# tuffy/libdvd-audio

Measured on AMD Instinct MI355X. Metric: decoded PCM Msamples/s (bit-exact) on 6ch/96k/24b MLP, higher is better.
Workload: dtype int32 (int64 accumulate)

## Files before the change

### libdvd-audio_amd/csrc/mlp_decode.h

```cpp
#pragma once
#include <hip/hip_runtime.h>
#if defined(__HIP_DEVICE_COMPILE__) && !defined(__gfx950__)
#error "mlp_decode.h is written for gfx950 (MI355X): hand-placed s_waitcnt encodings and gfx950 inline asm"
#endif
#include <stdint.h>
#include <type_traits>
#include "mlp_bounds.h"
#include "mlp_index.h"
#include "mlp_tables.h"

namespace mlp {

constexpr int DEC_THREADS = 128;
constexpr int DEC_WAVES = DEC_THREADS / 64;
constexpr int MAXCH = 8;
constexpr int MAXMAT = 6;
constexpr int RING_PLANES = 8;
constexpr int RING_DWORDS = RING_PLANES * 4;
constexpr int CHUNK_DWORDS = 16;
constexpr int OUT_ROWS = 4;
constexpr uint32_t YIELD_LONELY = 48;
#ifndef DVDA_HDR_GATE_TURNS
#define DVDA_HDR_GATE_TURNS 32
#endif
// ... 210 lines not shown

template <int RD>
__device__ __forceinline__ void ring_store4(uint32_t *dst, const uint4 &a, bool first_plane)
{
    const uint32_t a0 = be32(a.x);
    if (first_plane)
        dst[-RD * 64] = a0;
    dst[0] = a0;
    dst[-1 * 64] = be32(a.y);
    dst[-2 * 64] = be32(a.z);
    dst[-3 * 64] = be32(a.w);
}

__device__ __forceinline__ void ring_fill_sync(const uint4 *src, uint32_t *dst, bool first_plane)
{
    const uint4 a = src[0], b = src[1], c = src[2], d = src[3];
    ring_store16(dst, a, b, c, d, first_plane);
}

__device__ __attribute__((noinline)) int64_t iir_mac(const int32_t *ws, uint32_t stride)
{
    int64_t acc = 0;
    for (uint32_t j = 0; j < 8; j++)
        acc += (int64_t)ws[(size_t)j * stride] * (int64_t)ws[(size_t)(8 + j) * stride];
    return acc;
}

__device__ __attribute__((noinline)) void iir_push(int32_t *ws, uint32_t stride, int32_t v)
{
    for (int j = 7; j > 0; j--)
        ws[(size_t)(8 + j) * stride] = ws[(size_t)(8 + j - 1) * stride];
    ws[(size_t)8 * stride] = v;
}

template <int RD, int G>
struct BitReaderT {
    const uint4 *gsrc;
    uint32_t *ring;
    uint32_t max_chunk;
    uint32_t pos;
    uint32_t fillpos;
    uint32_t lo_valid;

    __device__ __forceinline__ uint32_t *slot(uint32_t d) const
    {
        return ring + ((RD - (d & (RD - 1))) << 6);
    }
    __device__ __forceinline__ uint64_t window() const
    {
        const uint32_t *p = ring + ((~(pos >> 5) & (RD - 1)) << 6);
        return ((uint64_t)p[64] << 32) | p[0];
    }
    __device__ __forceinline__ uint32_t window_lds() const
    {
        return (uint32_t)(uintptr_t)ring + ((~(pos >> 5) & (RD - 1)) << 8);
    }
    __device__ __forceinline__ int32_t ahead() const
    {
        return (int32_t)((fillpos << 5) - (pos & ~31u)) >> 5;
    }
    __device__ __forceinline__ void filled()
    {
        fillpos += G;
        if (fillpos - lo_valid > (uint32_t)RD)
            lo_valid = fillpos - RD;
    }
    __device__ __forceinline__ uint32_t fill_src() const
    {
        const uint32_t last = max_chunk + (uint32_t)(CHUNK_DWORDS - G);
        return fillpos < last ? fillpos : last;
    }
    __device__ __forceinline__ bool room() const { return ahead() <= (int32_t)(RD - G); }
    __device__ __forceinline__ void fill_sync()
    {
        if constexpr (G == CHUNK_DWORDS) {
            ring_fill_sync(gsrc + (fill_src() >> 2), slot(fillpos), (fillpos & (RD - 1)) == 0);
            filled();
        } else {
            uint4 q[4];
            const int32_t n = fill_issue(q);
            fill_commit(q, n);
        }
    }
    __device__ __forceinline__ int32_t fill_issue(uint4 (&q)[4]) const
    {
        static_assert(G == CHUNK_DWORDS || (G == 4 && RD == 16), "the small ring is 16 dwords filled by 16-byte granules");
        const int32_t n = room() ? (RD - ahead()) >> 2 : 0;
#pragma unroll
        for (int g = 0; g < 4; g++)
            if (g < n) {
                const uint32_t f = fillpos + 4u * g, last = max_chunk + (uint32_t)(CHUNK_DWORDS - G);
                q[g] = gsrc[(f < last ? f : last) >> 2];
            }
        return n;
    }
    __device__ __forceinline__ void fill_commit(const uint4 (&q)[4], int32_t n)
    {
#pragma unroll
        for (int g = 0; g < 4; g++)
            if (g < n) {
                ring_store4<RD>(slot(fillpos), q[g], (fillpos & (RD - 1)) == 0);
                filled();
            }
    }
    __device__ __forceinline__ void ensure(uint32_t n)
    {
#if defined(DVDA_EXP_STAMP)
        const unsigned long long t0_ = clock64();
        bool any_ = false;
#endif
        while (__builtin_expect(__any(ahead() < (int32_t)n), 0)) {
            if (room())
                fill_sync();
#if defined(DVDA_EXP_STAMP)
            any_ = true;
#endif
        }
#if defined(DVDA_EXP_STAMP)
        if (any_) {
            fill_cyc += clock64() - t0_;
            fill_n++;
        }
#endif
    }
#if defined(DVDA_EXP_STAMP)
    unsigned long long fill_cyc = 0, fill_n = 0;
#endif
    __device__ __forceinline__ void seek_byte(uint64_t byte_pos)
    {
        const uint32_t t = (uint32_t)(byte_pos >> 2);
        if (!((int32_t)(t - lo_valid) >= 0 && (int32_t)(fillpos - t) > 0)) {
            fillpos = t & ~(uint32_t)(G - 1);
            lo_valid = fillpos;
        }
        pos = (uint32_t)byte_pos << 3;
    }
    __device__ __forceinline__ uint64_t tell_near(uint64_t ref_bits) const
    {
        return ref_bits + (uint64_t)(int64_t)(int32_t)(pos - (uint32_t)ref_bits);
    }
    __device__ __forceinline__ bool past(uint32_t end_bits_lo) const { return (int32_t)(pos - end_bits_lo) > 0; }
    __device__ __forceinline__ uint32_t peek32()
    {
        ensure(2);
        return (uint32_t)((window() << (pos & 31u)) >> 32);
    }
    __device__ __forceinline__ uint32_t read(uint32_t n)
    {
        const uint32_t top = peek32();
        pos += n;
        return n ? top >> (32 - n) : 0u;
    }
    __device__ __forceinline__ uint32_t read_resident(uint32_t n)
    {
        const uint32_t top = (uint32_t)((window() << (pos & 31u)) >> 32);
        pos += n;
        return (top >> 1) >> (31u - n);
    }
    __device__ __forceinline__ int32_t read_signed_resident(uint32_t n)
    {
        const uint32_t top = (uint32_t)((window() << (pos & 31u)) >> 32);
        pos += n;
        return n ? (int32_t)top >> ((32u - n) & 31u) : 0;
    }
    __device__ __forceinline__ int32_t read_signed(uint32_t n)
    {
        if (n == 0)
            return 0;
        const int32_t v = (int32_t)peek32() >> (32 - n);
        pos += n;
        return v;
    }
};

using BitReader = BitReaderT<RING_DWORDS, CHUNK_DWORDS>;
constexpr int DUO_RING = 16, DUO_GRAN = 4;

__device__ __forceinline__ uint32_t huff_decode_m(uint32_t cb, uint32_t t, uint64_t m_esc, uint32_t bmask)
{
    const uint32_t a = (((t & 0xFFu) >> (5u + cb)) + 7u) | ((4u - cb) << 8);
    const uint32_t z = (uint32_t)__clz((int)((t << 25) | 0x01000000u));
    const uint32_t base = __builtin_amdgcn_ubfe(0x08090B08u, 8u * cb, 8u);
    uint32_t up = base + z, dn = 6u - z;
    asm volatile("" : "+v"(up), "+v"(dn));
    uint32_t val = (t & 0x80u) ? up : dn;
    val = z > 6u ? 0xFFu : val;
    uint32_t e = val | (((z > 6u ? 6u : z) + 3u) << 8);
    asm("v_cndmask_b32_e64 %0, %0, %1, %2" : "+v"(e) : "v"(a), "s"(m_esc));
    return e & bmask;
}

__device__ __forceinline__ uint32_t huff_decode(uint32_t cb, uint32_t t)
{
    uint64_t m_esc = __builtin_amdgcn_ballot_w64((t & 0x100u) != 0);
    asm volatile("" : "+s"(m_esc));
    return huff_decode_m(cb, t, m_esc, cb ? 0xFFFFFFFFu : 0u);
}

struct SubPark {
    uint32_t flags, block_size, min_ch, max_ch, max_mat_ch, noise_shift, seed, matrix_len, bypass_mask, outch_pack,
             oshift_pack, qss_pack, nslots, iir_any, ss_end_bit, rows_left, blocks_in_frame, chk, gl, seg_lane;
    bool have_restart, seg_iir;
    uint32_t *brec, *brec_end, *brec_base;
};

template <int NS, bool PAIRED, bool GENERAL, bool ILV = false, bool PARSE = false, bool DUO = false, bool WAVO = false>
__global__ __launch_bounds__(DEC_THREADS, 2) void k_decode(DecodeArgs a)
{
    static_assert(!(GENERAL && PARSE), "one mode at a time");
    static_assert(!DUO || (!PAIRED && !GENERAL && NS == 6), "the two-substream lane is a one-lane fast-pass / parse instance");
    static_assert(GENERAL == PAIRED, "lane pairs are the sequential pass's layout, and its only one");
    constexpr uint32_t L = PAIRED ? 2u : 1u;
    if (!GENERAL && a.only_S && a.cls[a.only_S - 1u] == 0)
        return;
    if (!GENERAL && !PARSE && coop_takes(a))
        return;
    constexpr int THREADS = DEC_THREADS;
    constexpr int WAVES = THREADS / 64;
    constexpr int TP = 6;
    constexpr int RD = DUO ? DUO_RING : RING_DWORDS;
    constexpr int RG = DUO ? DUO_GRAN : CHUNK_DWORDS;
    using Reader = BitReaderT<RD, RG>;
    __shared__ uint32_t s_ring[WAVES][DUO ? 2 : 1][RD + 1][64];
    __shared__ int32_t s_out[GENERAL ? 1 : WAVES][TP][OUT_ROWS][GENERAL ? 1 : 64];
    constexpr bool XCH = PAIRED;
    __shared__ int32_t s_xch[XCH ? WAVES : 1][MAXCH][XCH ? 64 : 1];
    __shared__ uint32_t s_nchained[WAVES];

    if (threadIdx.x < WAVES)
        s_nchained[threadIdx.x] = 0;
    __syncthreads();

    const int lane = threadIdx.x & 63;
    const int wv = threadIdx.x >> 6;
    const uint32_t wg_id = blockIdx.x;
    const uint32_t gl0 = wg_id * THREADS + threadIdx.x;
    uint32_t n_seg = *a.n_seg_ptr;
    if (n_seg > a.max_seg)
        n_seg = a.max_seg;
    const uint32_t item = gl0 / L;
    uint32_t segi = item;
    bool active = segi < n_seg;
    if (!GENERAL && !PARSE && active && *a.hetero)
        segi = DVDA_AT(a.lane_seg, item, a.caps.max_seg, BT_LANE_SEG);
    if (!GENERAL && !PARSE && segi >= n_seg) {
        active = false;
        segi = n_seg;
    }
    if (GENERAL || PARSE) {
        active = item < a.list_n && (a.list_n_ptr == nullptr || item < *a.list_n_ptr) && (!PARSE || item < DVDA_AT(a.plan, n_seg, a.caps.max_seg + 1u, BT_PLAN).y);
        segi = 0;
        if (active) {
            const uint32_t e = DVDA_AT(a.list, a.list_base + item, GENERAL ? a.caps.max_streams : a.caps.max_seg, BT_LIST);
            segi = GENERAL ? DVDA_AT(a.streams, e, a.caps.max_streams, BT_STREAMS).first_seg : e;
            active = segi < n_seg;
        }
        if (!active)
            segi = n_seg;
    }

    SegRec sr;
    sr.off = sr.end = 0;
    sr.stream = 0;
    sr.nframes = 0;
    sr.flags = 0;
    sr.sync = 0;
    sr.ndrop = 0;
    sr.prev = 0xFFFFFFFFu;
    uint32_t fbase = 0, stream_sync = 0, stream_first = 0;
    if (active) {
        sr = DVDA_AT(a.seg, segi, a.caps.max_seg, BT_SEG);
        stream_first = DVDA_AT(a.streams, sr.stream, a.caps.max_streams, BT_STREAMS).first_seg;
        if (stream_first == 0xFFFFFFFFu) {
            active = false;
            stream_first = segi;
        } else {
            stream_sync = a.streams[sr.stream].sync;
            fbase = a.seg_fbase[segi] - DVDA_AT(a.seg_fbase, stream_first, a.caps.max_seg + 1u, BT_FBASE);
        }
    }
    const uint32_t S = (stream_sync >> 24) & 0xF;
    const uint32_t sub = DUO ? 1u : gl0 - item * L;
    uint32_t gl = segi * 2u + sub;
    uint32_t seg_lane = gl;
    const uint32_t assignment = (stream_sync >> 16) & 0x1F;
    const uint32_t rpa = rows_per_au((stream_sync >> 8) & 0xF);
    const uint32_t nch_out = channel_count(assignment);
    const uint32_t wavepk = wave_pack(assignment);
    const uint32_t wave_inv = ILV ? wave_inv_pack(assignment) : 0u;
    uint32_t status = 0;
    if (active && (sr.flags & ST_FATAL_INDEX))
        active = false;
    if (active && (sub >= S || sr.nframes == 0))
        active = false;
    bool mine = GENERAL || !a.only_S || S == a.only_S;
    if (!mine)
        active = false;
    if (active && S > (DUO ? 2u : L)) {
        status |= ST_ENVELOPE;
        active = false;
    }
    if (DUO && S != 2u)
        active = false;
    if (active && (rpa == 0 || nch_out == 0)) {
        status |= ST_ENVELOPE;
        active = false;
    }
    const bool is_last_sub = (sub + 1 == S);
    const bool owner = is_last_sub;

// ... 62 lines not shown
        const uint64_t edge = out_stride < row_limit ? out_stride : row_limit;
        if (edge > row0)
            room = edge - row0 > 0xFFFFFFFFull ? 0xFFFFFFFFu : (uint32_t)(edge - row0);
    }
    const bool vec_ok = PARSE || ((((out_base | out_stride) & 3) == 0) &&
                                  ((reinterpret_cast<uintptr_t>(a.pcm) & 15) == 0));
    bool dir_ok = true;
    if (ILV && !GENERAL && !PARSE && segi < n_seg) {
        const uint64_t ob = a.out_off[sr.stream], os = a.out_stride[sr.stream];
        dir_ok = nch_out == 6u && (wavepk & 0xFFFFFFu) == 0x543210u && ((ob | os) & 3) == 0 &&
                 (reinterpret_cast<uintptr_t>(a.pcm) & 15) == 0;
    }
    const bool ilv_direct = ILV && !GENERAL && !PARSE && __all(dir_ok);

    Reader rd;
    rd.gsrc = reinterpret_cast<const uint4 *>(a.bytes);
    rd.ring = &s_ring[wv][DUO ? 1 : 0][0][lane];
    rd.max_chunk = (uint32_t)(((a.total_bytes + 63) >> 6) << 4);
    rd.pos = 0;
    rd.fillpos = 0;
    rd.lo_valid = 0;
    uint32_t chk = active ? DVDA_AT(a.seg_check, (size_t)segi * 2u + sub, 2ull * a.caps.max_seg, BT_CHECK) : 0xFFFFFFFFu;
    Reader rx;
    rx.gsrc = rd.gsrc;
    rx.ring = &s_ring[wv][0][0][lane];
    rx.max_chunk = rd.max_chunk;
    rx.pos = 0;
    rx.fillpos = 0;
    rx.lo_valid = 0;
    SubPark P0;
    P0.flags = 0xFF;
    P0.block_size = 8;
    P0.min_ch = P0.max_ch = P0.max_mat_ch = P0.noise_shift = P0.seed = P0.matrix_len = P0.bypass_mask = P0.outch_pack = 0;
    P0.oshift_pack = P0.qss_pack = P0.nslots = P0.iir_any = P0.ss_end_bit = P0.rows_left = P0.blocks_in_frame = 0;
    P0.have_restart = false;
    P0.seg_iir = false;
    P0.gl = segi * 2u;
    P0.seg_lane = P0.gl;
    P0.chk = (DUO && active) ? DVDA_AT(a.seg_check, (size_t)segi * 2u, 2ull * a.caps.max_seg, BT_CHECK) : 0xFFFFFFFFu;
    P0.brec = P0.brec_end = P0.brec_base = nullptr;
    if (DUO && PARSE && active) {
        const uint4 pl = DVDA_AT(a.plan, segi, a.caps.max_seg + 1u, BT_PLAN);
        P0.brec = a.brec + brec_offset(pl.x, pl.y, 0u, seg_R);
        P0.brec_base = P0.brec;
        P0.brec_end = P0.brec + brec_capacity(seg_R);
        if (!DVDA_RANGE_OK(brec_offset(pl.x, pl.y, 0u, seg_R), brec_capacity(seg_R), a.caps.brec, BT_BREC)) {
            status |= ST_CAPACITY;
            active = false;
        }
    }

    uint64_t sp[NS][4];
    auto st_get = [&](int k, int j) -> int32_t {
        return (j & 1) ? (int32_t)(uint32_t)(sp[k][j >> 1] >> 32) : (int32_t)(uint32_t)sp[k][j >> 1];
    };
    auto st_set = [&](int k, int j, int32_t v) {
        if (j & 1)
            sp[k][j >> 1] = (sp[k][j >> 1] & 0xFFFFFFFFull) | ((uint64_t)(uint32_t)v << 32);
        else
            sp[k][j >> 1] = (sp[k][j >> 1] & 0xFFFFFFFF00000000ull) | (uint32_t)v;
    };
    constexpr bool CFU = !PARSE && !GENERAL && !DUO;
    constexpr int CFW = CFU ? 8 : 4;
    int32_t cf[NS][CFW];
    uint32_t pk[NS];
    int32_t sho[NS];
    uint32_t mreg[2][4];
    uint32_t mnoise[2] = {0, 0};
    constexpr bool MU = ILV && !PAIRED && !GENERAL && !PARSE && !DUO;
    int32_t mu[2][MU ? 8 : 1];
#pragma unroll
    for (int m = 0; m < 2; m++)
#pragma unroll
        for (int j = 0; j < (MU ? 8 : 1); j++)
            mu[m][j] = 0;
#pragma unroll
    for (int k = 0; k < NS; k++) {
#pragma unroll
        for (int j = 0; j < 4; j++)
            sp[k][j] = 0;
#pragma unroll
        for (int j = 0; j < CFW; j++)
            cf[k][j] = 0;
        pk[k] = 24u << 2;
        sho[k] = -(1 << 23);
    }
#pragma unroll
    for (int m = 0; m < 2; m++)
#pragma unroll
        for (int j = 0; j < 4; j++)
            mreg[m][j] = 0;
    if (GENERAL && resume_from_init) {
#pragma unroll
        for (int k = 0; k < NS; k++)
#pragma unroll
            for (int j = 0; j < 8; j++)
                st_set(k, j, a.init_fir[((size_t)sr.stream * 2 + sub) * 48 + k * 8 + j]);
    }
    uint32_t flags = 0xFF;
    uint32_t block_size = 8;
    uint32_t min_ch = 0, max_ch = 0, max_mat_ch = 0, noise_shift = 0, seed = 0;
    uint32_t matrix_len = 0, bypass_mask = 0, outch_pack = 0;
    uint32_t oshift_pack = 0, qss_pack = 0;
    uint32_t qss_A = 0, mmc_A = 0;
    uint32_t gate_turn = 0;
    auto no_restart_yet = [&]() -> uint32_t {
        if (GENERAL)
            return ST_ENVELOPE;
        const uint32_t first = a.streams[a.seg[segi].stream].first_seg;
        return segi != first ? ST_SEQ : ST_ENVELOPE;
    };
    constexpr bool HDR_GATE = !PAIRED && !GENERAL;
    const uint32_t gl_r = gl;
    uint32_t nslots = 0;
    bool have_restart = false;
    uint32_t iir_any = 0;
    bool seg_iir = false;

    uint64_t cur = sr.off;
    uint32_t ss_end_bit = 0;
    uint32_t rows_left = 0;
    bool in_frame = false;
    uint32_t frame_rows = 0;
    uint32_t blocks_in_frame = 0;
    uint32_t frames_done = 0;
    uint64_t row = row0;
    uint32_t rows_written = 0;
    uint32_t rows_done = 0;
    int32_t pq_s[OUT_ROWS] = {0, 0, 0, 0};
    uint32_t au_idx = 0;
    uint32_t drops_seen = 0;
    uint32_t dsub = sub;
    auto swap_sub = [&]() {
        auto sw = [](uint32_t &x, uint32_t &y) { const uint32_t t = x; x = y; y = t; };
        auto swb = [](bool &x, bool &y) { const bool t = x; x = y; y = t; };
        auto swp = [](uint32_t *&x, uint32_t *&y) { uint32_t *const t = x; x = y; y = t; };
        sw(rd.pos, rx.pos);
        sw(rd.fillpos, rx.fillpos);
        sw(rd.lo_valid, rx.lo_valid);
        swp(rd.ring, rx.ring);
        sw(flags, P0.flags);
        sw(block_size, P0.block_size);
        sw(min_ch, P0.min_ch);
        sw(max_ch, P0.max_ch);
        sw(max_mat_ch, P0.max_mat_ch);
        sw(noise_shift, P0.noise_shift);
        sw(seed, P0.seed);
        sw(matrix_len, P0.matrix_len);
        sw(bypass_mask, P0.bypass_mask);
        sw(outch_pack, P0.outch_pack);
        sw(oshift_pack, P0.oshift_pack);
        sw(qss_pack, P0.qss_pack);
        sw(nslots, P0.nslots);
        sw(iir_any, P0.iir_any);
        sw(ss_end_bit, P0.ss_end_bit);
        sw(rows_left, P0.rows_left);
        sw(blocks_in_frame, P0.blocks_in_frame);
        sw(chk, P0.chk);
        sw(gl, P0.gl);
        sw(seg_lane, P0.seg_lane);
        swb(have_restart, P0.have_restart);
        swb(seg_iir, P0.seg_iir);
        swp(brec, P0.brec);
        swp(brec_end, P0.brec_end);
        swp(brec_base, P0.brec_base);
        dsub ^= 1u;
    };
// ... 342 lines not shown
                                            a.mat_ws[(size_t)(m * 5 + (c >> 1)) * a.total_lanes + gl] = word;
#pragma unroll
                                            for (int mm = 0; mm < 2; mm++)
#pragma unroll
                                                for (int jj = 0; jj < 4; jj++)
                                                    if ((uint32_t)mm == m && (uint32_t)jj == (c >> 1) && mat_mine) {
                                                        mreg[mm][jj] = word;
                                                        if constexpr (MU) {
                                                            if (jj < 3) {
                                                                mu[mm][MU ? 2 * jj : 0] = lo16(word);
                                                                mu[mm][MU ? 2 * jj + 1 : 0] = hi16(word);
                                                            }
                                                        }
                                                    }
                                        }
                                    } else {
                                        pair = (uint32_t)vc & 0xFFFFu;
                                    }
                                }
                                a.mat_ws[(size_t)(m * 5 + 4) * a.total_lanes + gl] = noise;
                                if (m == 0 && mat_mine)
                                    mnoise[0] = noise;
                                if (m == 1 && mat_mine)
                                    mnoise[1] = noise;
                                if constexpr (MU) {
#pragma unroll
                                    for (int mm = 0; mm < 2; mm++)
                                        if ((uint32_t)mm == m && mat_mine) {
                                            mu[mm][MU ? 6 : 0] = lo16(noise);
                                            mu[mm][MU ? 7 : 0] = hi16(noise);
                                        }
                                }
                            }
                        } else if (restart) {
                            matrix_len = 0;
                            bypass_mask = 0;
                        }
                        if (ok && (flags & 0x04u) && rd.read_resident(1)) {
                            if (blocks_in_frame)
                                matrix_class_change = true;
                            for (uint32_t c = 0; c <= max_mat_ch; c++) {
                                const int32_t v = rd.read_signed_resident(4);
                                if (v < 0) {
                                    ok = false;
                                    err = ST_ENVELOPE;
                                }
                                oshift_pack = (oshift_pack & ~(0xFu << (4 * c))) | (((uint32_t)v & 0xFu) << (4 * c));
                            }
                        } else if (restart) {
                            oshift_pack = 0;
                        }
                        bool qss_changed = false;
                        if (ok && (flags & 0x08u) && rd.read_resident(1)) {
                            if (blocks_in_frame)
                                matrix_class_change = true;
                            for (uint32_t c = 0; c <= max_ch; c++)
                                qss_pack = (qss_pack & ~(0xFu << (4 * c))) | (rd.read_resident(4) << (4 * c));
                            qss_changed = true;
                        } else if (restart) {
                            qss_pack = 0;
                            qss_changed = true;
                        }
                        DVDA_HSTAMP(2);
                        for (uint32_t k = 0; k < nslots && ok; k++) {
                            rd.ensure(HDR_FIR);
                            const uint32_t c = min_ch + k;
                            const uint32_t kr = DUO ? c : k;
                            uint32_t pk_old = 0;
                            int32_t sho_old = 0;
                            uint32_t cf_old[4] = {0, 0, 0, 0};
#pragma unroll
                            for (int kk = 0; kk < NS; kk++)
                                if ((uint32_t)kk == kr) {
                                    pk_old = pk[kk];
                                    sho_old = sho[kk];
                                    if (PARSE) {
#pragma unroll
                                        for (int j = 0; j < 4; j++)
                                            cf_old[j] = !CFU ? (uint32_t)cf[kk][CFU ? 0 : j]
                                                             : (((uint32_t)cf[kk][CFU ? 2 * j : 0] & 0xFFFFu) |
                                                                ((uint32_t)cf[kk][CFU ? 2 * j + 1 : 0] << 16));
                                    }
                                }
                            uint32_t codebook = pk_old & 3u;
                            const uint32_t lb_old = (pk_old >> 2) & 31u, q_old = (pk_old >> 7) & 15u;
                            uint32_t iir_order = (pk_old >> 15) & 0xFu, fir_order = (pk_old >> 19) & 0xFu;
                            uint32_t fir_shift = (pk_old >> 23) & 0xFu, iir_shift = (pk_old >> 27) & 0xFu;
                            uint32_t lsbs = lb_old + q_old;
                            int32_t hoff = sho_old + huff_center(codebook, lb_old);
                            bool touched = qss_changed;
                            bool new_fir = false, new_iir = false;
                            uint32_t ncf[4] = {0, 0, 0, 0};
                            if (rd.read_resident(1)) {
                                touched = true;
                                if ((flags & 0x10u) && rd.read_resident(1)) {
                                    fir_order = rd.read_resident(4);
                                    new_fir = true;
                                    if (fir_order > 8) {
                                        ok = false;
                                    } else if (fir_order == 0) {
                                        fir_shift = 0;
                                    } else {
                                        fir_shift = rd.read_resident(4);
                                        const uint32_t cbits = rd.read_resident(5);
                                        const uint32_t cshift = rd.read_resident(3);
                                        if (cbits < 1 || cbits > 16 || cbits + cshift > 16) {
                                            ok = false;
                                        } else {
#pragma unroll
                                            for (int j = 0; j < 8; j++) {
                                                int32_t v = 0;
                                                if ((uint32_t)j < fir_order)
                                                    v = (int32_t)((uint32_t)rd.read_signed_resident(cbits) << cshift);
                                                if (j & 1)
                                                    ncf[j >> 1] |= (uint32_t)v << 16;
                                                else
                                                    ncf[j >> 1] = (uint32_t)v & 0xFFFFu;
                                            }
                                            if (rd.read_resident(1))
                                                ok = false;
                                        }
                                    }
                                } else if (restart) {
                                    fir_order = 0;
                                    fir_shift = 0;
                                    new_fir = true;
                                }
                                rd.ensure(HDR_IIR);
                                if (ok && (flags & 0x20u) && rd.read_resident(1)) {
                                    new_iir = true;
                                    iir_order = rd.read_resident(4);
                                    if (iir_order > 8) {
                                        ok = false;
                                    } else if (iir_order == 0) {
                                        iir_shift = 0;
                                    } else {
                                        iir_shift = rd.read_resident(4);
                                        const uint32_t cbits = rd.read_resident(5);
                                        const uint32_t cshift = rd.read_resident(3);
                                        if (cbits < 1 || cbits > 16 || cbits + cshift > 16) {
                                            ok = false;
                                        } else {
                                            int32_t *ws = a.iir_ws + (size_t)(k * 16) * a.total_lanes + gl;
                                            for (uint32_t j = 0; j < 8; j++) {
                                                int32_t v = 0;
                                                if (j < iir_order)
                                                    v = (int32_t)((uint32_t)rd.read_signed_resident(cbits) << cshift);
                                                ws[(size_t)j * a.total_lanes] = v;
                                            }
                                            rd.ensure(HDR_IIR_STATE);
                                            if (rd.read_resident(1)) {
                                                const uint32_t sbits = rd.read_resident(4), sshift = rd.read_resident(4);
                                                if (sbits == 0) {
                                                    ok = false;
                                                    err = ST_ENVELOPE;
                                                }
                                                for (uint32_t j = 0; j < 8; j++) {
                                                    int32_t v = 0;
                                                    if (j < iir_order)
                                                        v = (int32_t)((uint32_t)rd.read_signed_resident(sbits) << sshift);
                                                    ws[(size_t)(8 + j) * a.total_lanes] = v;
                                                }
                                            } else {
                                                ok = false;
                                                err = ST_ENVELOPE;
                                            }
                                        }
                                    }
                                } else if (restart) {
                                    new_iir = true;
                                    iir_order = 0;
                                    iir_shift = 0;
                                }
                                if (ok && (flags & 0x40u) && rd.read_resident(1))
                                    hoff = rd.read_signed_resident(15);
                                else if (restart)
                                    hoff = 0;
                                codebook = rd.read_resident(2);
                                lsbs = rd.read_resident(5);
                                if (lsbs > 24)
                                    ok = false;
                            } else if (restart) {
                                touched = true;
                                fir_order = fir_shift = iir_order = iir_shift = 0;
                                new_fir = true;
                                new_iir = true;
                                hoff = 0;
                                codebook = 0;
                                lsbs = 24;
                            }
                            if (touched && ok) {
                                const uint32_t q = nib(qss_pack, c);
                                if (lsbs < q) {
                                    ok = false;
                                    err = ST_ENVELOPE;
                                } else {
                                    const uint32_t lb = lsbs - q;
                                    uint32_t shift;
                                    if (fir_order + iir_order > 8) {
                                        ok = false;
                                        err = ST_FILTER;
                                    }
                                    if (fir_shift > 0 && iir_shift > 0) {
                                        if (fir_shift != iir_shift) {
                                            ok = false;
                                            err = ST_FILTER;
                                        }
                                        shift = fir_shift;
                                    } else if (fir_order > 0) {
                                        shift = fir_shift;
                                    } else {
                                        shift = iir_shift;
                                    }
                                    if (fir_order && frames_done == 0 && blocks_in_frame == 0)
                                        status |= ST_CHAINED;
                                    const int32_t nsho = hoff - huff_center(codebook, lb);
                                    const uint32_t npk = codebook | (lb << 2) | (q << 7) | (shift << 11) |
                                                         (iir_order << 15) | (fir_order << 19) |
                                                         (fir_shift << 23) | (iir_shift << 27) |
                                                         (codebook ? 1u << 31 : 0u);
#pragma unroll
                                    for (int kk = 0; kk < NS; kk++)
                                        if ((uint32_t)kk == kr) {
                                            pk[kk] = npk;
                                            sho[kk] = nsho;
                                            if (new_fir) {
#pragma unroll
                                                for (int j = 0; j < 4; j++) {
                                                    if constexpr (!CFU) {
                                                        cf[kk][CFU ? 0 : j] = (int32_t)ncf[j];
                                                    } else {
                                                        cf[kk][CFU ? 2 * j : 0] = lo16(ncf[j]);
                                                        cf[kk][CFU ? 2 * j + 1 : 0] = hi16(ncf[j]);
                                                    }
                                                }
                                            }
                                        }
                                    iir_any = (iir_any & ~(1u << k)) | ((iir_order ? 1u : 0u) << k);
                                    if (PARSE) {
                                        const bool with_iir = new_iir && iir_order != 0;
                                        if (brec + 2 * BREC_STRIDE + (with_iir ? BREC_IIR_WORDS : 0) > brec_end) {
                                            seq_needed = true;
                                        } else {
                                            uint32_t *w = brec + BREC_SLOT * k;
                                            w[2] = shift | (q << 4) | (fir_order << 8) | (iir_order << 12) |
                                                   (new_iir ? 1u << 16 : 0u);
#pragma unroll
                                            for (int j = 0; j < 4; j++)
                                                w[3 + j] = new_fir ? ncf[j] : cf_old[j];
                                            w[7] = 0;
                                            chg_mask |= 1u << k;
                                            if (with_iir) {
                                                const int32_t *ws = a.iir_ws + (size_t)(k * 16) * a.total_lanes + gl;
                                                brec_end -= BREC_IIR_WORDS;
                                                uint32_t *x = brec_end;
                                                for (uint32_t j = 0; j < 4; j++)
                                                    x[j] = ((uint32_t)ws[(size_t)(2 * j) * a.total_lanes] & 0xFFFFu) |
                                                           ((uint32_t)ws[(size_t)(2 * j + 1) * a.total_lanes] << 16);
                                                for (uint32_t j = 0; j < 8; j++)
                                                    x[4 + j] = (uint32_t)ws[(size_t)(8 + j) * a.total_lanes];
                                                w[7] = (uint32_t)(x - brec_base);
                                            }
                                        }
                                    }
                                }
                            }
                        }
                    }
                }
                DVDA_HSTAMP(3);
                if (!have_restart && ok) {
                    ok = false;
                    err = no_restart_yet();
                }
                hdr_parsed = true;
                if (PARSE && iir_any)
                    seg_iir = true;
                if (PARSE && ok && chg_mask) {
#pragma unroll
                    for (int kk = 0; kk < 6; kk++) {
                        brec[BREC_SLOT * kk] = rows_done;
                        brec[BREC_SLOT * kk + 1] = (chg_mask >> kk) & 1u;
                    }
                    brec += BREC_STRIDE;
                }
                if (PARSE && ok && (seq_needed || (hdr_restart && blocks_in_frame))) {
                    status |= ST_SEQ;
                    active = false;
                }
                if (mat_mine) {
                    qss_A = qss_pack;
                    mmc_A = max_mat_ch;
                }
                const uint32_t cold_ml = matrix_len;
                if (matrix_class_change)
                    status |= ST_MIDFRAME;
                if (!ok) {
                    status |= err;
                    active = false;
                } else if (PARSE && !active) {
                } else if (!GENERAL && !PARSE && (iir_any != 0 || cold_ml > 2)) {
                    status |= ST_COLD;
                    active = false;
                } else if (!GENERAL && !PARSE && (status & ST_CHAINED)) {
                    active = false;
                    if (!(DUO && probe))
                        atomicAdd(&s_nchained[wv], 1u);
                    if (sr.prev != 0xFFFFFFFFu)
                        __hip_atomic_store(&DVDA_AT(a.yield_req, sr.prev, a.caps.max_seg, BT_YIELD), 1u, __ATOMIC_RELAXED, __HIP_MEMORY_SCOPE_AGENT);
                } else {
                    rows_left = block_size;
                    blocks_in_frame++;
                    if (!GENERAL && !PARSE && frames_done < 2 &&
                        __hip_atomic_load(&s_nchained[wv], __ATOMIC_RELAXED, __HIP_MEMORY_SCOPE_WORKGROUP) >= YIELD_LONELY) {
                        status |= ST_YIELD;
                        active = false;
                    }
                }
            }
                if constexpr (DUO) {
                    if (pass == 0u && me)
                        swap_sub();
                    if (!PARSE && pass == 0u && me && !active && first0 && !(status & ~ST_INFO)) {
                        probe = true;
                        active = true;
                    }
                    if (pass == 1u && probe)
                        active = false;
                }
            }
            if constexpr (DUO) {
                if (active && have_restart && P0.have_restart && (P0.min_ch != 0u || min_ch != P0.max_ch + 1u)) {
                    status |= PARSE ? ST_SEQ : ST_COLD;
                    active = false;
                }
            }
        }
        if (hdr_now) {
            DVDA_HSTAMP(4);
#if defined(DVDA_EXP_STAMP)
            hstamp_acc[5] += rd.fill_cyc + (DUO ? rx.fill_cyc : 0ull);
            hfills += rd.fill_n + (DUO ? rx.fill_n : 0ull);
            hcount++;
#endif
        }
        if (!__any(active))
            break;
        DVDA_STAMP(0);

        if (active) {
            if constexpr (DUO) {
                while (__builtin_expect(__any(rd.ahead() < 8 || rx.ahead() < 8), 0)) {
                    DVDA_COV(14);
                    uint4 q0[4], q1[4];
                    const int32_t n0 = rx.fill_issue(q0), n1 = rd.fill_issue(q1);
                    rx.fill_commit(q0, n0);
                    rd.fill_commit(q1, n1);
                }
            } else {
            if (rd.ahead() < 12)
                DVDA_COV(14);
            rd.ensure(12);
            }
        }
        DVDA_STAMP(7);
        const bool pf = active && rd.room();
        const bool pfx = DUO && active && rx.room();
        uint4 p0, p1, p2, p3;
        asm volatile("" : "=v"(p0.x), "=v"(p0.y), "=v"(p0.z), "=v"(p0.w), "=v"(p1.x), "=v"(p1.y), "=v"(p1.z), "=v"(p1.w),
                          "=v"(p2.x), "=v"(p2.y), "=v"(p2.z), "=v"(p2.w), "=v"(p3.x), "=v"(p3.y), "=v"(p3.z), "=v"(p3.w));
        bool flush = false;
        const uint32_t frames_before = frames_done;
        uint64_t flush_row = 0;
        if constexpr (DUO) {
            if (pfx)
                p0 = rx.gsrc[rx.fill_src() >> 2];
            if (pf)
                p1 = rd.gsrc[rd.fill_src() >> 2];
        } else {
        if (pf) {
            const uint32_t c = rd.fillpos < rd.max_chunk ? rd.fillpos : rd.max_chunk;
            const uint4 *src = rd.gsrc + (c >> 2);
            p0 = src[0];
            p1 = src[1];
            p2 = src[2];
            p3 = src[3];
        }
        }
        DVDA_STAMP(1);

        uint32_t bypass_bits = 0;
        int32_t val[NS];
        auto row_head_any = [&]() {
            if (__any(bypass_mask != 0)) {
                const uint32_t cnt = (uint32_t)__popc(bypass_mask);
                const uint32_t field = rd.read_resident(cnt);
                const uint32_t b0 = bypass_mask & 1u, b1 = (bypass_mask >> 1) & 1u;
                bypass_bits = (b0 & (field >> ((cnt - 1u) & 31u))) | ((b1 & (field >> ((cnt - 1u - b0) & 31u))) << 1);
                if ((GENERAL || PARSE) && __builtin_expect(__any((bypass_mask >> 2) != 0), 0)) {
                    if (bypass_mask >> 2)
                        DVDA_COV(10);
                    uint32_t rank = b0 + b1;
#pragma unroll
                    for (int m = 2; m < MAXMAT; m++) {
                        const uint32_t bit = (bypass_mask >> m) & 1u;
                        bypass_bits |= (bit & (field >> ((cnt - 1u - rank) & 31u))) << m;
                        rank += bit;
                    }
                }
            }
            if constexpr (DUO)
                rx.pos += (uint32_t)__popc(P0.bypass_mask);
            uint32_t cpos = DUO ? rx.pos : rd.pos;
            uint32_t cbase = (uint32_t)(uintptr_t)(DUO ? rx.ring : rd.ring);
            auto cur_window_lds = [&]() -> uint32_t { return cbase + ((~(cpos >> 5) & (uint32_t)(RD - 1)) << 8); };
            uint64_t win = DUO ? rx.window() : rd.window();
            const uint32_t n_sub0 = DUO ? P0.max_ch + 1u : 0u;
            uint32_t msb_or = 0;
            const bool wave_iir = GENERAL && __any(iir_any != 0);
#pragma unroll
            for (int k = 0; k < NS; k++) {
                const bool in = DUO ? (uint32_t)k <= max_ch : (uint32_t)k < nslots;
                if (k > 0)
                    asm volatile("s_waitcnt lgkmcnt(0)" : "+v"(win));
                if constexpr (DUO) {
                    if (k > 0) {
                        const bool sw = (uint32_t)k == n_sub0;
                        if (__any(sw)) {
                            if (sw) {
                                rx.pos = cpos;
                                cpos = rd.pos;
                                cbase = (uint32_t)(uintptr_t)rd.ring;
                                win = rd.window();
                            }
                        }
                    }
                }
                val[k] = 0;
                if (k >= 2 && !__any(in))
                    continue;
                if (in) {
                const uint32_t pkk = pk[k];
                const uint32_t cb = pkk & 3u, lb = (pkk >> 2) & 31u, q = (pkk >> 7) & 15u,
                               shift = (pkk >> 11) & 15u;
                const uint32_t bmask = (uint32_t)((int32_t)pkk >> 31);
                const uint32_t ofs = cpos & 31u;
                const uint32_t top = (uint32_t)((win << ofs) >> 32);
                uint64_t m_esc = __builtin_amdgcn_ballot_w64((int32_t)top < 0);
                asm volatile("" : "+s"(m_esc));
                const uint32_t e = huff_decode_m(cb, top >> 23, m_esc, bmask);
                const uint32_t msb = e & 0xFFu;
                const uint32_t len = e >> 8;
                msb_or |= msb;
                const uint32_t o2 = ofs + len;
                cpos += len + lb;
                const uint32_t top2 = (uint32_t)((win << o2) >> 32);
                const uint32_t lsbv = (top2 >> 1) >> (31u - lb);
                if (k + 1 < NS)
                    asm volatile("ds_read2st64_b32 %0, %2 offset1:1" : "+v"(win), "+v"(sp[k][0]) : "v"(cur_window_lds()));
                const int32_t residual = (int32_t)(((msb << lb) + lsbv + (uint32_t)sho[k]) << q);
                int32_t value;
                if constexpr (PARSE) {
                    value = residual;
                    (void)shift;
                    (void)wave_iir;
                } else {
                auto tap = [&](int j) -> int32_t {
                    if constexpr (CFU)
                        return cf[k][CFU ? j : 0];
                    else
                        return (j & 1) ? hi16((uint32_t)cf[k][CFU ? 0 : j >> 1]) : lo16((uint32_t)cf[k][CFU ? 0 : j >> 1]);
                };
                int64_t acc0 = (int64_t)tap(0) * (int64_t)st_get(k, 0);
                int64_t acc1 = (int64_t)tap(1) * (int64_t)st_get(k, 1);
                acc0 += (int64_t)tap(2) * (int64_t)st_get(k, 2);
                acc1 += (int64_t)tap(3) * (int64_t)st_get(k, 3);
                acc0 += (int64_t)tap(4) * (int64_t)st_get(k, 4);
                acc1 += (int64_t)tap(5) * (int64_t)st_get(k, 5);
                acc0 += (int64_t)tap(6) * (int64_t)st_get(k, 6);
                acc1 += (int64_t)tap(7) * (int64_t)st_get(k, 7);
                int64_t acc = acc0 + acc1;
                bool iir_on = false;
                if (__builtin_expect(wave_iir, 0)) {
                    iir_on = in && ((iir_any >> k) & 1u);
                    if (iir_on)
                        DVDA_COV(11);
                    if (iir_on)
                        acc += iir_mac(a.iir_ws + (size_t)(k * 16) * a.total_lanes + gl, a.total_lanes);
                }
                const int32_t ssum = (int32_t)(acc >> shift);
                value = mask_q((int32_t)((uint32_t)ssum + (uint32_t)residual), q);
                {
                    const uint64_t vpair = (uint64_t)(uint32_t)value;
                    asm("v_pk_mov_b32 %0, %1, %0 op_sel:[1,0]" : "+v"(sp[k][3]) : "v"(sp[k][2]));
                    asm("v_pk_mov_b32 %0, %1, %0 op_sel:[1,0]" : "+v"(sp[k][2]) : "v"(sp[k][1]));
                    asm("v_pk_mov_b32 %0, %1, %0 op_sel:[1,0]" : "+v"(sp[k][1]) : "v"(sp[k][0]));
                    asm("v_pk_mov_b32 %0, %1, %0 op_sel:[0,0]" : "+v"(sp[k][0]) : "v"(vpair));
                }
                if (__builtin_expect(wave_iir, 0)) {
                    if (iir_on)
                        iir_push(a.iir_ws + (size_t)(k * 16) * a.total_lanes + gl, a.total_lanes,
                                 (int32_t)((uint32_t)value - (uint32_t)ssum));
                }
                }
                val[k] = value;
                }
            }
            rd.pos = cpos;
            if (__builtin_expect((msb_or & 0x80u) != 0, 0)) {
                status |= ST_HUFFMAN;
                active = false;
            }
            DVDA_STAMP(2);
        };
        auto row_tail = [&](int32_t (&ch)[MAXCH]) {
            if (owner) {
                if (GENERAL) {
                    if (frame_rows >= (uint32_t)FB_ROWS) {
                        status |= ST_ENVELOPE;
                        active = false;
                    } else {
                        int32_t *fr = fbuf + (size_t)frame_rows * (MAXCH + 1);
#pragma unroll
                        for (int c = 0; c < MAXCH; c++)
                            fr[c] = ch[c];
                        fr[MAXCH] = (int32_t)bypass_bits;
                    }
                } else {
                    if constexpr (PARSE) {
#pragma unroll
                        for (int j = 0; j < OUT_ROWS - 1; j++) {
                            pq_s[j] = pq_s[j + 1];
                        }
                        pq_s[OUT_ROWS - 1] = (int32_t)((seed & 0x7FFFFFu) | (bypass_bits << 23));
                        const uint32_t shifted = (seed >> 7) & 0xFFFFu;
                        seed = (seed << 16) ^ shifted ^ (shifted << 5);
                    } else {
                        rematrix(ch, bypass_bits);
                    }
                    const uint32_t ph = rows_done & (OUT_ROWS - 1);
                    int32_t(*T)[OUT_ROWS][GENERAL ? 1 : 64] =
                        s_out[GENERAL ? 0 : wv];
                    if (ILV && ilv_direct) {
                        int32_t *Td = &T[0][0][GENERAL ? 0 : lane] + ph * (6 * 64);
#pragma unroll
                        for (int c = 0; c < 6; c++)
                            Td[c * 64] = ch[c];
                    } else {
#pragma unroll
                        for (int c = 0; c < TP; c++)
                            T[c][ph][GENERAL ? 0 : lane] = ch[c];
                    }
                    if (__builtin_expect(room == 0, 0)) {
                        if (row >= out_stride && row < row_limit) {
                            status |= ST_OVERFLOW;
                            active = false;
                        }
                    } else {
                        rows_written++;
                        if (ph == OUT_ROWS - 1) {
                            flush = true;
                            flush_row = row - (OUT_ROWS - 1);
                        }
                    }
                }
            }
            row++;
            rows_done++;
            if (GENERAL) {
                if (row > row_limit) {
                    status |= ST_TIMING;
                    active = false;
                }
            } else if (__builtin_expect(room == 0, 0)) {
                if (row > row_limit) {
                    status |= ST_TIMING;
                    active = false;
                }
            } else {
                room--;
            }
            frame_rows++;
            rows_left--;
            if constexpr (DUO) {
                P0.rows_left--;
// ... 536 lines not shown
```

Measured before the change: 239,500.

## Repack per-channel hot params and make Huffman decode branch- and ballot-free

Splits the per-channel packed parameter word into a hot word, holding codebook-derived constants, lb, q and a combined shift+q, and a cold 16-bit word kept in LDS for the filter orders and shifts. The Huffman decoder now works directly on the top window bits with mask arithmetic instead of a wave ballot and cndmask. Residual and prediction are combined with a single left shift by q that replaces mask_q. The DUO refill loop now fills one granule per reader per iteration, and the LDS window address computation is simplified. These changes aim to cut VALU/SALU instructions in the per-sample inner loop, at the cost of extra LDS traffic on the parameter-change path and subtler bit-exactness conditions.

Result: faster. 250,800 (median of 6 runs) (+4.7%).

```diff
diff --git a/libdvd-audio_amd/csrc/mlp_decode.h b/libdvd-audio_amd/csrc/mlp_decode.h
--- a/libdvd-audio_amd/csrc/mlp_decode.h
+++ b/libdvd-audio_amd/csrc/mlp_decode.h
@@ -316,22 +316,26 @@
             fill_commit(q, n);
         }
     }
-    __device__ __forceinline__ int32_t fill_issue(uint4 (&q)[4]) const
+    template <int MAXG = 4>
+    __device__ __forceinline__ int32_t fill_issue(uint4 (&q)[MAXG]) const
     {
         static_assert(G == CHUNK_DWORDS || (G == 4 && RD == 16), "the small ring is 16 dwords filled by 16-byte granules");
-        const int32_t n = room() ? (RD - ahead()) >> 2 : 0;
-#pragma unroll
-        for (int g = 0; g < 4; g++)
+        int32_t n = room() ? (RD - ahead()) >> 2 : 0;
+        if (MAXG < 4 && n > MAXG)
+            n = MAXG;
+#pragma unroll
+        for (int g = 0; g < MAXG; g++)
             if (g < n) {
                 const uint32_t f = fillpos + 4u * g, last = max_chunk + (uint32_t)(CHUNK_DWORDS - G);
                 q[g] = gsrc[(f < last ? f : last) >> 2];
             }
         return n;
     }
-    __device__ __forceinline__ void fill_commit(const uint4 (&q)[4], int32_t n)
+    template <int MAXG = 4>
+    __device__ __forceinline__ void fill_commit(const uint4 (&q)[MAXG], int32_t n)
     {
 #pragma unroll
-        for (int g = 0; g < 4; g++)
+        for (int g = 0; g < MAXG; g++)
             if (g < n) {
                 ring_store4<RD>(slot(fillpos), q[g], (fillpos & (RD - 1)) == 0);
                 filled();
@@ -410,25 +414,41 @@
 using BitReader = BitReaderT<RING_DWORDS, CHUNK_DWORDS>;
 constexpr int DUO_RING = 16, DUO_GRAN = 4;
 
-__device__ __forceinline__ uint32_t huff_decode_m(uint32_t cb, uint32_t t, uint64_t m_esc, uint32_t bmask)
+__host__ __device__ constexpr uint32_t hot_word(uint32_t cb, uint32_t lb, uint32_t q, uint32_t shift)
 {
-    const uint32_t a = (((t & 0xFFu) >> (5u + cb)) + 7u) | ((4u - cb) << 8);
-    const uint32_t z = (uint32_t)__clz((int)((t << 25) | 0x01000000u));
-    const uint32_t base = __builtin_amdgcn_ubfe(0x08090B08u, 8u * cb, 8u);
-    uint32_t up = base + z, dn = 6u - z;
-    asm volatile("" : "+v"(up), "+v"(dn));
-    uint32_t val = (t & 0x80u) ? up : dn;
-    val = z > 6u ? 0xFFu : val;
-    uint32_t e = val | (((z > 6u ? 6u : z) + 3u) << 8);
-    asm("v_cndmask_b32_e64 %0, %0, %1, %2" : "+v"(e) : "v"(a), "s"(m_esc));
-    return e & bmask;
+    return lb | (q << 5) | ((shift + q) << 10) |
+           (cb ? ((7u - (8u >> cb)) << 16) | ((cb == 1 ? 9u : cb == 2 ? 7u : 6u) << 20) | ((4u - cb) << 24) |
+                 ((28u + cb) << 26) | (1u << 31)
+               : 0u);
+}
+__device__ __forceinline__ uint32_t hot_cb(uint32_t hw) { return (hw >> 26) & 3u; }
+__device__ __forceinline__ uint32_t hot_lb(uint32_t hw) { return hw & 31u; }
+__device__ __forceinline__ uint32_t hot_q(uint32_t hw) { return (hw >> 5) & 15u; }
+__host__ __device__ constexpr uint32_t cold_word(uint32_t iir_order, uint32_t fir_order, uint32_t fir_shift, uint32_t iir_shift)
+{
+    return iir_order | (fir_order << 4) | (fir_shift << 8) | (iir_shift << 12);
+}
+
+__device__ __forceinline__ uint32_t huff_decode_top(uint32_t top, uint32_t hw)
+{
+    const uint32_t a = (top >> ((hw >> 26) & 31u)) + ((hw >> 16) & 0x307u);
+    const uint32_t n = (uint32_t)__clz((int)((top & 0x3F800000u) | 0x00400000u));
+    const uint32_t up = ((hw >> 20) & 0x10Fu) + n, dn = 0x108u - n;
+    uint32_t d = 0x40000000u - (top & 0x7F800000u);
+    asm("" : "+v"(d));
+    uint32_t ms = (uint32_t)((int32_t)d >> 31);
+    asm("" : "+v"(ms));
+    uint32_t val = (up & ms) | (dn & ~ms);
+    asm("" : "+v"(val));
+    const uint32_t e = (n << 8) + val;
+    uint32_t m = (uint32_t)((int32_t)top >> 31);
+    asm("" : "+v"(m));
+    return ((a & m) | (e & ~m)) & (uint32_t)((int32_t)hw >> 31);
 }
 
 __device__ __forceinline__ uint32_t huff_decode(uint32_t cb, uint32_t t)
 {
-    uint64_t m_esc = __builtin_amdgcn_ballot_w64((t & 0x100u) != 0);
-    asm volatile("" : "+s"(m_esc));
-    return huff_decode_m(cb, t, m_esc, cb ? 0xFFFFFFFFu : 0u);
+    return huff_decode_top(t << 23, hot_word(cb, 0u, 0u, 0u));
 }
 
 struct SubPark {
@@ -460,6 +480,7 @@
     constexpr bool XCH = PAIRED;
     __shared__ int32_t s_xch[XCH ? WAVES : 1][MAXCH][XCH ? 64 : 1];
     __shared__ uint32_t s_nchained[WAVES];
+    __shared__ uint16_t s_cold[WAVES][NS][64];
 
     if (threadIdx.x < WAVES)
         s_nchained[threadIdx.x] = 0;
@@ -688,7 +709,8 @@
 #pragma unroll
         for (int j = 0; j < CFW; j++)
             cf[k][j] = 0;
-        pk[k] = 24u << 2;
+        pk[k] = hot_word(0u, 24u, 0u, 0u);
+        s_cold[wv][k][lane] = (uint16_t)cold_word(0u, 0u, 0u, 0u);
         sho[k] = -(1 << 23);
     }
 #pragma unroll
@@ -1197,10 +1219,12 @@
                                                                 ((uint32_t)cf[kk][CFU ? 2 * j + 1 : 0] << 16));
                                     }
                                 }
-                            uint32_t codebook = pk_old & 3u;
-                            const uint32_t lb_old = (pk_old >> 2) & 31u, q_old = (pk_old >> 7) & 15u;
-                            uint32_t iir_order = (pk_old >> 15) & 0xFu, fir_order = (pk_old >> 19) & 0xFu;
-                            uint32_t fir_shift = (pk_old >> 23) & 0xFu, iir_shift = (pk_old >> 27) & 0xFu;
+                            uint32_t codebook = hot_cb(pk_old);
+                            const uint32_t lb_old = hot_lb(pk_old), q_old = hot_q(pk_old);
+                            uint16_t *const cold = &s_cold[wv][kr < (uint32_t)NS ? kr : 0u][lane];
+                            const uint32_t cold_old = kr < (uint32_t)NS ? *cold : 0u;
+                            uint32_t iir_order = cold_old & 0xFu, fir_order = (cold_old >> 4) & 0xFu;
+                            uint32_t fir_shift = (cold_old >> 8) & 0xFu, iir_shift = (cold_old >> 12) & 0xFu;
                             uint32_t lsbs = lb_old + q_old;
                             int32_t hoff = sho_old + huff_center(codebook, lb_old);
                             bool touched = qss_changed;
@@ -1330,10 +1354,9 @@
                                     if (fir_order && frames_done == 0 && blocks_in_frame == 0)
                                         status |= ST_CHAINED;
                                     const int32_t nsho = hoff - huff_center(codebook, lb);
-                                    const uint32_t npk = codebook | (lb << 2) | (q << 7) | (shift << 11) |
-                                                         (iir_order << 15) | (fir_order << 19) |
-                                                         (fir_shift << 23) | (iir_shift << 27) |
-                                                         (codebook ? 1u << 31 : 0u);
+                                    const uint32_t npk = hot_word(codebook, lb, q, shift);
+                                    if (kr < (uint32_t)NS)
+                                        *cold = (uint16_t)cold_word(iir_order, fir_order, fir_shift, iir_shift);
 #pragma unroll
                                     for (int kk = 0; kk < NS; kk++)
                                         if ((uint32_t)kk == kr) {
@@ -1467,10 +1490,11 @@
             if constexpr (DUO) {
                 while (__builtin_expect(__any(rd.ahead() < 8 || rx.ahead() < 8), 0)) {
                     DVDA_COV(14);
-                    uint4 q0[4], q1[4];
-                    const int32_t n0 = rx.fill_issue(q0), n1 = rd.fill_issue(q1);
-                    rx.fill_commit(q0, n0);
-                    rd.fill_commit(q1, n1);
+                    uint4 q[1];
+                    const int32_t n0 = rx.template fill_issue<1>(q);
+                    rx.template fill_commit<1>(q, n0);
+                    const int32_t n1 = rd.template fill_issue<1>(q);
+                    rd.template fill_commit<1>(q, n1);
                 }
             } else {
             if (rd.ahead() < 12)
@@ -1527,8 +1551,8 @@
             if constexpr (DUO)
                 rx.pos += (uint32_t)__popc(P0.bypass_mask);
             uint32_t cpos = DUO ? rx.pos : rd.pos;
-            uint32_t cbase = (uint32_t)(uintptr_t)(DUO ? rx.ring : rd.ring);
-            auto cur_window_lds = [&]() -> uint32_t { return cbase + ((~(cpos >> 5) & (uint32_t)(RD - 1)) << 8); };
+            uint32_t cbase = (uint32_t)(uintptr_t)(DUO ? rx.ring : rd.ring) + (uint32_t)((RD - 1) << 8);
+            auto cur_window_lds = [&]() -> uint32_t { return cbase - ((cpos << 3) & (uint32_t)((RD - 1) << 8)); };
             uint64_t win = DUO ? rx.window() : rd.window();
             const uint32_t n_sub0 = DUO ? P0.max_ch + 1u : 0u;
             uint32_t msb_or = 0;
@@ -1545,7 +1569,7 @@
                             if (sw) {
                                 rx.pos = cpos;
                                 cpos = rd.pos;
-                                cbase = (uint32_t)(uintptr_t)rd.ring;
+                                cbase = (uint32_t)(uintptr_t)rd.ring + (uint32_t)((RD - 1) << 8);
                                 win = rd.window();
                             }
                         }
@@ -1555,29 +1579,27 @@
                 if (k >= 2 && !__any(in))
                     continue;
                 if (in) {
-                const uint32_t pkk = pk[k];
-                const uint32_t cb = pkk & 3u, lb = (pkk >> 2) & 31u, q = (pkk >> 7) & 15u,
-                               shift = (pkk >> 11) & 15u;
-                const uint32_t bmask = (uint32_t)((int32_t)pkk >> 31);
+                const uint32_t hw = pk[k];
+                const uint32_t lb = hw & 31u;
                 const uint32_t ofs = cpos & 31u;
                 const uint32_t top = (uint32_t)((win << ofs) >> 32);
-                uint64_t m_esc = __builtin_amdgcn_ballot_w64((int32_t)top < 0);
-                asm volatile("" : "+s"(m_esc));
-                const uint32_t e = huff_decode_m(cb, top >> 23, m_esc, bmask);
+                const uint32_t e = huff_decode_top(top, hw);
                 const uint32_t msb = e & 0xFFu;
                 const uint32_t len = e >> 8;
                 msb_or |= msb;
                 const uint32_t o2 = ofs + len;
                 cpos += len + lb;
                 const uint32_t top2 = (uint32_t)((win << o2) >> 32);
-                const uint32_t lsbv = (top2 >> 1) >> (31u - lb);
+                const uint32_t lsbv = (top2 >> 1) >> (~hw & 31u);
                 if (k + 1 < NS)
                     asm volatile("ds_read2st64_b32 %0, %2 offset1:1" : "+v"(win), "+v"(sp[k][0]) : "v"(cur_window_lds()));
-                const int32_t residual = (int32_t)(((msb << lb) + lsbv + (uint32_t)sho[k]) << q);
+                uint32_t ml = (msb << (hw & 31u)) + lsbv;
+                asm("" : "+v"(ml));
+                const uint32_t resq = ml + (uint32_t)sho[k];
+                const uint32_t q5 = (hw >> 5) & 31u;
                 int32_t value;
                 if constexpr (PARSE) {
-                    value = residual;
-                    (void)shift;
+                    value = (int32_t)(resq << q5);
                     (void)wave_iir;
                 } else {
                 auto tap = [&](int j) -> int32_t {
@@ -1603,19 +1625,22 @@
                     if (iir_on)
                         acc += iir_mac(a.iir_ws + (size_t)(k * 16) * a.total_lanes + gl, a.total_lanes);
                 }
-                const int32_t ssum = (int32_t)(acc >> shift);
-                value = mask_q((int32_t)((uint32_t)ssum + (uint32_t)residual), q);
+                value = (int32_t)(((uint32_t)(acc >> ((hw >> 10) & 63u)) + resq) << q5);
                 {
-                    const uint64_t vpair = (uint64_t)(uint32_t)value;
+                    uint32_t vhi;
+                    asm("" : "=v"(vhi));
+                    const uint64_t vpair = (uint64_t)(uint32_t)value | ((uint64_t)vhi << 32);
                     asm("v_pk_mov_b32 %0, %1, %0 op_sel:[1,0]" : "+v"(sp[k][3]) : "v"(sp[k][2]));
                     asm("v_pk_mov_b32 %0, %1, %0 op_sel:[1,0]" : "+v"(sp[k][2]) : "v"(sp[k][1]));
                     asm("v_pk_mov_b32 %0, %1, %0 op_sel:[1,0]" : "+v"(sp[k][1]) : "v"(sp[k][0]));
                     asm("v_pk_mov_b32 %0, %1, %0 op_sel:[0,0]" : "+v"(sp[k][0]) : "v"(vpair));
                 }
                 if (__builtin_expect(wave_iir, 0)) {
-                    if (iir_on)
+                    if (iir_on) {
+                        const int32_t ssum = (int32_t)(acc >> (((hw >> 10) & 63u) - hot_q(hw)));
                         iir_push(a.iir_ws + (size_t)(k * 16) * a.total_lanes + gl, a.total_lanes,
                                  (int32_t)((uint32_t)value - (uint32_t)ssum));
+                    }
                 }
                 }
                 val[k] = value;
```
